# zhenxuan00/graphical-gan

Hardware: AMD Instinct MI355X
Metric: images/sec (G+D+GP step) cifar10 32x32 bs=64 (higher is better)
Workload: dtype f32; 1 GPU; gan_inference_cifar10.py MODE=wali-gp BATCH_SIZE=64 (per GPU) 32x32x3, CRITIC_ITERS=5; parallelism=dp1, global_batch=64, hip_graph=True, minibatch_feed=device-resident ring, read in place; one graph per iteration, finite_costs=True

## Files before the change

graphical_gan_amd/_lib.py:

```python
import ctypes as C
import os

_HERE = os.path.dirname(os.path.abspath(__file__))
LIB_PATH = os.path.join(_HERE, 'libggan.so')

ACT_NONE, ACT_LRELU, ACT_RELU, ACT_TANH, ACT_SIGMOID = 0, 1, 2, 3, 4
PACK_MAX = 64
HEAD_BCE_MAX_ROWS = 2048
BCE_HEADS = 2
PACK_ARRIVE_INTS = 33 * 1024
POSTERIOR_MAX_K = 8192
MODE_K = {'CONCRETE': 0, 'STRAIGHT_THROUGHT_CONCRETE': 1, 'STRAIGHT_THROUGHT': 2}
BCE_MAX = 16
TSNE_MAX_K = 128
TSNE_MAX_SPLITS = 64
ABI_VERSION = 800


class ConvGeom(C.Structure):
    _fields_ = [(n, C.c_int) for n in ('N', 'Ci', 'H', 'W', 'Co', 'Ho', 'Wo', 'k', 'stride', 'pad_t', 'pad_l',
                                       'plan_wgs', 'plan_wgs_filter', 'plan_flags')]


PLAN_PLAIN = 1
# ... 58 lines not shown
    'ggan_ssim_pairs_workspace': (_Z, [_I, _I, _I, _I]),
    'ggan_ssim_pairs': (_I, [_P, _P, _I, _I, _I, _I, _F, _F, _F, _F, _P, _P, _P, _Z, _P]),
    'ggan_noise_fill': (_I, [_P, _P, _P, _P, _P, _P, _I, _P, _P]),
    'ggan_gmm_latent_fwd': (_I, [_P, _P, _P, _P, _P, _I, _I, _I, _F, _F, _P]),
    'ggan_gmm_latent_bwd': (_I, [_P, _P, _P, _P, _P, _P, _P, _I, _I, _I, _F, _P]),
    'ggan_gmm_latent_st_fwd': (_I, [_P, _P, _P, _P, _P, _P, _I, _I, _I, _F, _F, _I, _P]),
    'ggan_gmm_latent_st_bwd': (_I, [_P, _P, _P, _P, _P, _P, _P, _I, _I, _I, _F, _I, _P]),
    'ggan_gmm_posterior_assign': (_I, [_P, _P, _F, _I, _I, _I, _I, _P, _P, _P, _P]),
    'ggan_cluster_accuracy': (_I, [_P, _P, _P, _I, _I, _P, _P]),
    'ggan_video_sheet_u8': (_I, [_P, _P, _P, _P, _I, _I, _I, _I, _I, _I, _I, _I, _I, _F, _F, _F, _P]),
    'ggan_tsne_sqnorms': (_I, [_P, _I, _I, _P, _P]),
    'ggan_tsne_neighbours': (_I, [_P, _P, _I, _I, _I, _I, _I, _P, _P, _P, _P, _Z, _P]),
    'ggan_tsne_affinities': (_I, [_P, _I, _I, _F, _I, _F, _P, _P, _P]),
    'ggan_tsne_symmetrise': (_I, [_P, _P, _I, _I, _P, _P, _P, _P, _P]),
    'ggan_tsne_gradient': (_I, [_P, _P, _P, _P, _I, _I, _P, _P, _P, _P, _P, _P]),
    'ggan_tsne_kl': (_I, [_P, _P, _P, _P, _I, _I, _P, _P, _P, _P, _P]),
    'ggan_tsne_iterate': (_I, [_P, _P, _P, _P, _P, _P, _P, _I, _I, _P, _P, _I, _I, _I, _F, _F, _F, _F, _F, _P]),
    'ggan_gemm_split': (_I, [_I, _I, _I, _I, _I, _P, _P, _I, _P, _P, _P, _P, _I, _P, _I, _F, _P, _Z, _P]),
    'ggan_gemm_colsum': (_I, [_I, _I, _I, _I, _P, _P, _P, _P, _P, _Z, _P]),
    'ggan_dyn_scan_fwd': (_I, [_I, _I, _I, _I, _I, _P, _P, _P, _P, _P, _P, _P, _P, _P, _P, _F, _P, _P, _P, _P]),
    'ggan_dyn_scan_bwd': (_I, [_I, _I, _I, _I, _I, _P, _P, _P, _P, _P, _P, _P, _P, _P, _F, _P, _P, _P, _P, _P, _P, _P]),
    'ggan_critic_head_fwd': (_I, [_I, _I, _I, _I, _P, _P, _P, _P, _P, _P, _F, _P, _P, _P, _Z, _P]),
    'ggan_critic_head_bwd': (_I, [_I, _I, _I, _I, _P, _P, _P, _P, _P, _P, _F, _P, _P, _P, _P, _P, _P, _P, _P, _Z, _P]),
    'ggan_critic_head_fwd_bce': (_I, [_I, _I, _I, _I, _P, _P, _P, _P, _P, _P, _F, _P, _P, _I, _I, _P, _P, _P, _P, _P, _P, _Z, _P]),
    'ggan_critic_head_bwd_tail': (_I, [_I, _I, _I, _I, _P, _P, _P, _P, _P, _F, _P, _P, _P, _P, _P, _P, _P, _P, _P, _I, _I, _P, _P, _P, _P, _P, _P, _Z, _P]),
    'ggan_linear_bwd_data_act': (_I, [_I, _I, _I, _P, _P, _I, _F, _P, _P, _P, _Z, _P]),
    'ggan_linear_bwd_weight_act': (_I, [_I, _I, _I, _P, _P, _P, _I, _F, _P, _P, _P, _Z, _P]),
    'ggan_colsum': (_I, [_P, _P, _I, _I, _P]),
    'ggan_reparam_fwd': (_I, [_P, _P, _P, _P, _P, _Z, _P]),
    'ggan_reparam_bwd': (_I, [_P, _P, _P, _P, _P, _P, _Z, _P]),
    'ggan_agg_div_fwd': (_I, [_I, _P, _P, _P, _P, _P, _I, _I, _I, _I, _P, _P, _P, _P, _P, _P]),
    'ggan_agg_div_bwd': (_I, [_I, _P, _P, _P, _P, _I, _I, _I, _I, _P, _P, _P, _P, _P, _P, _P, _P, _P]),
    'ggan_colsum_tall': (_I, [_P, _P, _I, _I, _P, _Z, _P]),
    'ggan_chansum': (_I, [_P, _P, _I, _I, _I, _P, _Z, _P]),
    'ggan_bn_fwd_train': (_I, [_P, _P, _P, _P, _P, _P, _I, _I, _I, _F, _I, _F, _P]),
    'ggan_bn_bwd': (_I, [_P, _P, _P, _P, _P, _P, _P, _P, _I, _I, _I, _P]),
    'ggan_bn_bwd_act': (_I, [_P, _P, _P, _I, _F, _P, _P, _P, _P, _P, _P, _P, _I, _I, _I, _P]),
    'ggan_bn_bwd_bwd': (_I, [_P, _P, _P, _I, _F, _P, _P, _P, _P, _P, _P, _P, _I, _I, _I, _P]),
    'ggan_bn_split_fwd_train': (_I, [_P, _P, _P, _P, _P, _P, _I, _I, _I, _I, _F, _I, _F, _P, _Z, _P]),
    'ggan_bn_split_bwd_act': (_I, [_P, _P, _I, _F, _P, _P, _P, _P, _P, _P, _P, _P, _I, _I, _I, _I, _I, _P, _Z, _P]),
    'ggan_bn_sync_stats': (_I, [_P, _P, _I, _I, _I, _P]),
    'ggan_bn_sync_apply': (_I, [_P, _P, _I, _P, _P, _P, _P, _P, _I, _I, _I, _F, _I, _F, _P]),
    'ggan_bn_sync_bwd_stats': (_I, [_P, _P, _P, _I, _F, _P, _P, _P, _I, _I, _I, _P]),
    'ggan_bn_sync_bwd_apply': (_I, [_P, _P, _P, _I, _F, _P, _P, _P, _P, _I, _I, _P, _P, _P, _I, _I, _I, _P]),
    'ggan_act_fwd': (_I, [_P, _P, _Z, _I, _F, _P]),
    'ggan_act_bwd': (_I, [_P, _P, _P, _Z, _I, _F, _P]),
    'ggan_act_bwd_chansum': (_I, [_P, _P, _P, _P, _I, C.POINTER(_I), _I, _I, _I, _I, _F, _P]),
    'ggan_bias_add': (_I, [_P, _P, _P, _I, _I, _I, _P]),
    'ggan_cast_scale_i32': (_I, [_P, _P, _P, _Z, _F, _F, _P]),
    'ggan_cast_scale_ring_i32': (_I, [_P, _I, _P, _P, _I, _P, _P, _Z, _F, _F, _P]),
    'ggan_axpby': (_I, [_P, _P, _P, _Z, _F, _F, _F, _P]),
    'ggan_mix_mean': (_I, [_P, _P, _P, _P, _I, _I, _I, _P]),
    'ggan_row_lerp': (_I, [_P, _P, _P, _P, _I, _I, _P]),
    'ggan_bce_logits_fwd': (_I, [_P, _F, _F, _P, _I, _I, _P]),
    'ggan_bce_logits_bwd': (_I, [_P, _F, _F, _P, _P, _I, _P]),
    'ggan_bce_logits_multi_fwd': (_I, [C.POINTER(_P), C.POINTER(_F), C.POINTER(_F), C.POINTER(_I), _I, _P, _P]),
    'ggan_bce_logits_multi_bwd': (_I, [C.POINTER(_P), C.POINTER(_F), C.POINTER(_F), C.POINTER(_I), _I, _P, C.POINTER(_P), _P]),
    'ggan_bce_logits_multi_fwd_grad': (_I, [C.POINTER(_P), C.POINTER(_F), C.POINTER(_F), C.POINTER(_I), _I, _P, C.POINTER(_P), _P]),
    'ggan_bce_head_bwd': (_I, [C.POINTER(_P), C.POINTER(_F), C.POINTER(_F), C.POINTER(_I), _I, _P, C.POINTER(_P), _I, _I, _P, _P, _F, _P, _P,
                          _P, _P]),
    'ggan_bce_heads_bwd': (_I, [C.POINTER(_P), C.POINTER(_F), C.POINTER(_F), C.POINTER(_I), _I, _P, C.POINTER(_P), _I, C.POINTER(_I),
                           C.POINTER(_I), C.POINTER(_I), C.POINTER(_P), C.POINTER(_P), C.POINTER(_F), C.POINTER(_P), C.POINTER(_P),
                           C.POINTER(_P), _P]),
    'ggan_mean_fwd': (_I, [_P, _F, _P, _I, _I, _P]),
    'ggan_mean_bwd': (_I, [_P, _F, _P, _I, _P]),
    'ggan_mean_multi_fwd_grad': (_I, [C.POINTER(_P), C.POINTER(_F), C.POINTER(_I), _I, _P, C.POINTER(_P), _P]),
    'ggan_dist_fwd': (_I, [_P, _P, _P, _Z, _I, _F, _I, _P]),
    'ggan_dist_bwd': (_I, [_P, _P, _P, _P, _P, _Z, _I, _F, _P]),
    'ggan_gp_penalty_fwd': (_I, [_P, _P, _P, _I, _I, _F, _P]),
    'ggan_gp_penalty_bwd': (_I, [_P, _P, _P, _P, _I, _I, _F, _P]),
    'ggan_gp_penalty_fwd_grad': (_I, [_P, _P, _P, _P, _P, _I, _I, _F, _P]),
    'ggan_adam_step': (_I, [_P, _P, _P, _P, _Z, _P, _F, _F, _F, _F, _F, _P]),
    'ggan_adam_advance': (_I, [_P, _P]),
    'ggan_rmsprop_step': (_I, [_P, _P, _P, _Z, _F, _F, _F, _F, _F, _F, _P]),
    'ggan_adam_step_counted': (_I, [_P, _P, _P, _P, _Z, _P, _F, _F, _F, _F, _F, _P]),
    'ggan_ema_step': (_I, [_P, _P, _Z, _P, _F, _P]),
    'ggan_swap': (_I, [_P, _P, _Z, _P]),
    'ggan_pack': (_I, [C.POINTER(_P), C.POINTER(_Z), C.POINTER(_Z), _I, _P, _P]),
    'ggan_pack_parts': (_I, [C.POINTER(_P), C.POINTER(_Z), C.POINTER(_Z), C.POINTER(_I), C.POINTER(_Z), _I, _P, _P, _P]),
    'ggan_pack_parts2': (_I, [C.POINTER(_P), C.POINTER(_Z), C.POINTER(_Z), C.POINTER(_I), C.POINTER(_Z), C.POINTER(_P), C.POINTER(_I),
                              C.POINTER(_Z), _I, _P, _P, _P]),
    'ggan_pack_adam': (_I, [C.POINTER(_P), C.POINTER(_Z), C.POINTER(_Z), C.POINTER(_I), C.POINTER(_Z), C.POINTER(_P), C.POINTER(_I),
                            C.POINTER(_Z), _I, _P, _P, _P, _P, _P, _P, _F, _F, _F, _F, _F, _P]),
    'ggan_prof_enable': (_I, [_I]),
    'ggan_prof_reset': (_I, []),
    'ggan_prof_report': (_I, [C.POINTER(ProfRec), _I]),
}

_lib = None


def load():
    global _lib
    if _lib is not None:
        return _lib
    if not os.path.exists(LIB_PATH):
        raise GganError('libggan.so not found at %s -- run `python -c "import __graft_entry__ as g; g.build()"` '
                        '(there is no CPU fallback)' % LIB_PATH)
    lib = C.CDLL(LIB_PATH)
    for name, (res, args) in SIGNATURES.items():
        try:
            fn = getattr(lib, name)
        except AttributeError:
            raise GganError('libggan.so does not export %s' % name)
        fn.restype = res
        fn.argtypes = args
# ... 24 lines not shown
```

graphical_gan_amd/build.py:

```python
import hashlib
import os
import subprocess
import sys

HERE = os.path.dirname(os.path.abspath(__file__))
CSRC = os.path.join(HERE, 'csrc')
LIB = os.path.join(HERE, 'libggan.so')
STAMP = os.path.join(HERE, '.libggan.stamp')
SOURCES = ['runtime.hip', 'pointwise.hip', 'bn.hip', 'linear_bn.hip', 'gemm.hip', 'conv_naive.hip', 'conv_corr.hip', 'conv_dg16.hip', 'conv_wgrad.hip', 'conv_wgrad_split.hip', 'conv_thin.hip', 'conv_api.hip', 'conv3d.hip', 'dynscan.hip', 'video_sheet.hip', 'tsne.hip', 'mmd_sets.hip', 'knn_sets.hip', 'knn_lists.hip', 'parzen_sets.hip', 'ssim_pairs.hip']
FLAGS = ['--offload-arch=gfx950', '-O3', '-std=c++17', '-fPIC', '-ffp-contract=on', '-Wall', '-Wno-unused-function']
EXTRA_FLAGS = {'conv_wgrad_split.hip': ['-mllvm', '-amdgpu-mfma-vgpr-form']}
if os.environ.get('GGAN_BUILD_DIAG'):
    FLAGS.append('-DGGAN_DIAG')


def _digest():
    h = hashlib.sha256()
    for root in (CSRC, os.path.join(HERE, '..', 'include')):
        for fn in sorted(os.listdir(root)):
            with open(os.path.join(root, fn), 'rb') as f:
                h.update(fn.encode())
                h.update(f.read())
    h.update(' '.join(FLAGS).encode())
    h.update(repr(sorted(EXTRA_FLAGS.items())).encode())
    return h.hexdigest()


def build_id():
    h = hashlib.sha256()
    try:
        with open(os.path.join(HERE, 'site_plans.json'), 'rb') as f:
            h.update(f.read())
    except OSError:
        pass
    return _digest()[:16] + '/' + h.hexdigest()[:8]


def build(force=False, verbose=False):
    import fcntl
    with open(os.path.join(HERE, '.libggan.lock'), 'w') as lock:
        fcntl.flock(lock, fcntl.LOCK_EX)
        try:
            return _build_locked(force, verbose)
        finally:
            fcntl.flock(lock, fcntl.LOCK_UN)


def _build_locked(force, verbose):
    dig = _digest()
    if not force and os.path.exists(LIB) and os.path.exists(STAMP) and open(STAMP).read().strip() == dig:
        return LIB
    hipcc = os.environ.get('HIPCC', '/opt/rocm/bin/hipcc')
    objs = []
    procs = []
    for src in SOURCES:
        obj = os.path.join(HERE, 'build', src.replace('.hip', '.o'))
        os.makedirs(os.path.dirname(obj), exist_ok=True)
        cmd = [hipcc] + FLAGS + EXTRA_FLAGS.get(src, []) + ['-c', os.path.join(CSRC, src), '-o', obj]
        if verbose:
            print(' '.join(cmd))
        procs.append((src, subprocess.Popen(cmd, stdout=subprocess.PIPE, stderr=subprocess.STDOUT)))
        objs.append(obj)
# ... 22 lines not shown
```

graphical_gan_amd/functional/__init__.py:

```python

from ._core import (
    C, os, weakref, torch, Function, once_differentiable, _lib, ACT_NONE, ACT_LRELU, ACT_RELU, ACT_TANH, ACT_SIGMOID, ConvGeom,
    check, _WS, _WS_BYTES, _L, _p, _stream, _dev, _c, _DEFER, _DATA_ONLY, _is_param, data_grad_only,
    _skip_undefined, defer_wgrad_reduce, _wgrad_parts, _STREAMS, shared_stream, workspace, _PLAN, _PLAIN, _SERIAL_BWD, target_workgroups,
    launch_hint, serial_backward, _remembers_plan, force_plain,
    same_geometry, conv_geom, _geom, _SITE, site_scope, site_plan, RowSlot, _new_out, _adjacent, HEAD_LOGITS, _PENDING_COSTS, _tail_value, settle_cost,
    pending_costs, drop_pending_costs, UNIT_SEEDS, unit_seed, is_unit_seed, LATE_EXT, _LATE_TERMS, mark_ready, wait_ready, add_late_terms,
    drop_late_terms)
from .pointwise import ActFwd, ActBwd, leaky_relu, relu, tanh, sigmoid
from .conv import (
    DEBUG_POISON_CHECK, PendingCast, ConvFwd, _fused_conv_backward, ConvDgrad, ConvDgradMasked, ConvWgrad, ChanSum, TALL_ROWS,
    ColSum)
from .linear import (
    Gemm, _fused_linear_backward, Gemm2, _CONSTS, cached_const, Gemm2Dgrad, _HEAD_HINT, head_bce_hint, CriticHead, DynScan,
    gemm_colsum_, linear)
from .norm import BatchNormTrain, BatchNormGroupedTrain, BatchNormBwd, LinearBatchNormRows, _all_gather_rows, SyncBatchNormTrain
from .rows import (
    JoinRows, Fanout, fanout, SplitRows, CastScaleI32, Axpby, MixMean, GmmLatent, GmmLatentST, MixRbfMmd2, MixRbfMmd2Unbiased, mix_rbf_sums, mmd2_from_sums, MMD_FUSED_MAX_ROWS, knn_radii, ball_counts, prdc, PRDC_MAX_K, knn_lists, knn_vote, knn_accuracy, KNN_MAX_K, KNN_MAX_CLASSES, parzen_lse, parzen_ll, PARZEN_MAX_SIGMAS, ssim_pairs, psnr_from_mse, Reparam, AGG_KL, AGG_IKL, AGG_JSD,
    AggDiv, RowLerp, gmm_posterior_assign_, cluster_accuracy_, sheet_grid, video_sheet_u8)
from .conv3d import _dims3, Im2Col3d, Col2Im3d, _conv3d_patch, _igemm_ok, Conv3dImplicit, conv3d
from .losses import BceSum, Distance, MeanSum, GradPenalty
from .optim_ops import ema_step_, swap_
from .optim_ops import adam_step_, rmsprop_step_, NOISE_NORMAL, NOISE_UNIFORM, NOISE_ONEHOT, noise_state, noise_fill_, pack_
from .tsne import (
    tsne, tsne_splits, tsne_neighbours, tsne_affinities, tsne_symmetrise, tsne_gradient, tsne_kl, tsne_step, tsne_affinity_graph)
```

graphical_gan_amd/functional/linear.py:

```python
import ctypes as C
import os
import threading as _threading
import torch
import weakref
from .. import _lib
from torch.autograd import Function
from torch.autograd.function import once_differentiable
from .._lib import ACT_NONE, check
from ._core import (
    _L, _p, _stream, _c, _DATA_ONLY, _is_param, _skip_undefined, workspace, _new_out, HEAD_LOGITS, _PENDING_COSTS,
    _tail_value)
from .pointwise import ActBwd
from .conv import TALL_ROWS, ColSum


@_skip_undefined
class Gemm(Function):

    @staticmethod
    def forward(ctx, a, b, bias, ta, tb, act, alpha, slot=None):
        a, b = _c(a), _c(b)
        M, K = (a.shape[1], a.shape[0]) if ta else (a.shape[0], a.shape[1])
        K2, N = (b.shape[1], b.shape[0]) if tb else (b.shape[0], b.shape[1])
        assert K == K2, (a.shape, b.shape, ta, tb)
# ... 123 lines not shown

_CONSTS = {}


def cached_const(value, shape, device):
    device = torch.device(device)
    key = (float(value), tuple(shape), device.type, device.index)
    t = _CONSTS.get(key)
    if t is None:
        t = _CONSTS[key] = torch.full(tuple(shape), float(value), dtype=torch.float32, device=device)
    return t


class Gemm2Dgrad(Function):

    @staticmethod
    def forward(ctx, g, w, K1):
        g, w = _c(g), _c(w)
        M, N = g.shape
        K = w.shape[0]
        da1 = torch.empty((M, K1), dtype=torch.float32, device=g.device)
        da2 = torch.empty((M, K - K1), dtype=torch.float32, device=g.device)
        ws = workspace(g.device)
        check(_L().ggan_gemm_split(0, 1, M, K, N, _p(g), _p(None), 0, _p(w), _p(None), _p(da1), _p(da2), K1, _p(None), ACT_NONE, 0.0,
                                   _p(ws), ws.numel(), _stream()), 'ggan_gemm_split')
        ctx.K1 = K1
        ctx.w_param = _is_param(w)
        ctx.set_materialize_grads(False)
        ctx.save_for_backward(g, w)
        return da1, da2

    @staticmethod
    def backward(ctx, h1, h2):
        if h1 is None and h2 is None:
            return None, None, None
        g, w = ctx.saved_tensors
        K1 = ctx.K1
        M, N = g.shape
        K = w.shape[0]
        h1 = _c(h1) if h1 is not None else cached_const(0.0, (M, K1), g.device)
        h2 = _c(h2) if h2 is not None else cached_const(0.0, (M, K - K1), g.device)
        dg = dw = None
        if ctx.needs_input_grad[0]:
            dg = Gemm2.apply(h1, h2, w, None, ACT_NONE, 0.0)
        if ctx.needs_input_grad[1] and not (_DATA_ONLY[0] and ctx.w_param):
            if torch.is_grad_enabled():
                dw = Gemm.apply(torch.cat([h1, h2], 1), g, None, True, False, ACT_NONE, 0.0)
            else:
                dw = torch.empty((K, N), dtype=torch.float32, device=g.device)
                ws = workspace(g.device)
                check(_L().ggan_gemm_split(1, 0, K, N, M, _p(h1), _p(h2), K1, _p(g), _p(None), _p(dw), _p(None), 0, _p(None), ACT_NONE,
                                           0.0, _p(ws), ws.numel(), _stream()), 'ggan_gemm_split')
        return dg, dw, None


_HEAD_HINT = _threading.local()


class head_bce_hint(object):

    def __init__(self, terms, kind='bce'):
        self.terms = (kind, tuple((int(n), float(z), float(w)) for n, z, w in terms)) if terms else None

    def __enter__(self):
        self.prev = getattr(_HEAD_HINT, 'terms', None)
        _HEAD_HINT.terms = self.terms
        return self

    def __exit__(self, *exc):
        _HEAD_HINT.terms = self.prev
        return False


@_skip_undefined
class CriticHead(Function):

    @staticmethod
    def forward(ctx, a1, a2, w, b, w_out, b_out, alpha):
        a1, w, b, w_out, b_out = _c(a1), _c(w), _c(b), _c(w_out), _c(b_out)
        a2 = _c(a2) if a2 is not None else None
        M, K1 = a1.shape
        K2 = a2.shape[1] if a2 is not None else 0
        H = w.shape[1]
        assert w.shape[0] == K1 + K2 and w_out.numel() == H and b.numel() == H, (a1.shape, w.shape, w_out.shape)
        h = torch.empty((M, H), dtype=torch.float32, device=a1.device)
        logits = torch.empty((M,), dtype=torch.float32, device=a1.device)
        ws = workspace(a1.device)
        registers = M <= _lib.HEAD_BCE_MAX_ROWS and any(ctx.needs_input_grad) and not os.environ.get('GGAN_NO_HEAD_BCE')
        hint = getattr(_HEAD_HINT, 'terms', None)
        hinted = None
        hkind, hterms = hint if hint is not None else (None, ())
        if (registers and hint is not None and 1 <= len(hterms) <= 3 and sum(n for n, _, _ in hterms) == M and H <= 2048
                and not os.environ.get('GGAN_NO_HEAD_HINT')):
            g = torch.empty((M,), dtype=torch.float32, device=a1.device)
            gh = torch.empty((M, H), dtype=torch.float32, device=a1.device)
            nt = len(hterms)
            tabs = ((C.c_int * nt)(*[n for n, _, _ in hterms]), (C.c_float * nt)(*[z for _, z, _ in hterms]),
                    (C.c_float * nt)(*[wt for _, _, wt in hterms]))
            check(_L().ggan_critic_head_fwd_bce(M, K1, K2, H, _p(a1), _p(a2), _p(w), _p(b), _p(w_out), _p(b_out), float(alpha), _p(h),
                                                _p(logits), 1 if hkind == 'mean' else 0, nt, tabs[0], tabs[1], tabs[2], _p(g), _p(gh), _p(ws),
                                                ws.numel(), _stream()), 'ggan_critic_head_fwd_bce')
            hinted = dict(kind=hkind, terms=hterms, g=g, gh=gh)
        else:
            check(_L().ggan_critic_head_fwd(M, K1, K2, H, _p(a1), _p(a2), _p(w), _p(b), _p(w_out), _p(b_out), float(alpha), _p(h),
                                            _p(logits), _p(ws), ws.numel(), _stream()), 'ggan_critic_head_fwd')
        ctx.alpha, ctx.has_a2 = float(alpha), a2 is not None
# ... 123 lines not shown
```

graphical_gan_amd/models.py:

```python
import contextlib
import os
import weakref

import numpy as np
import torch

from . import functional as F
from . import tflib as lib
from .tflib.ops.act import LRELU, RELU, TANH, SIGMOID

NETS_TARGET_WGS = 128
GP_TARGET_WGS = 128


class Config(object):
    def __init__(self, dataset='cifar10', batch_size=64, n_coms=0, mode=None, dim=None, dim_latent=128, bn=None,
                 temp=0.1, fuse=True, lr=None, batch_critic=True, mode_k='CONCRETE'):
        self.dataset, self.B, self.K, self.dim_latent, self.temp, self.fuse = dataset, batch_size, n_coms, dim_latent, temp, fuse
        assert mode_k in ('CONCRETE', 'STRAIGHT_THROUGHT_CONCRETE', 'STRAIGHT_THROUGHT'), mode_k
        self.mode_k = mode_k
        if dataset == 'cifar10':
            self.C, self.S, self.dim, self.nl, self.bn, self.out_act = 3, 32, 64, 3, True, 'tanh'
        elif dataset == 'svhn':
            self.C, self.S, self.dim, self.nl, self.bn, self.out_act = 3, 32, 64, 3, False, 'tanh'
# ... 158 lines not shown
            out = self._bn('Generator.BN1', [0], out, RELU)
        else:
            out = self._lin('Generator.Input', c.dim_latent, c.flat, noise, RELU)
        slot = out_slot
        out = out.reshape(-1, c.top, 4, 4)
        names = ['2', '3', '4', '5'] if c.nl == 4 else ['2', '3', '5']
        ch = c.top
        for i, nm in enumerate(names):
            last = i == len(names) - 1
            cout = c.C if last else ch // 2
            final_act = TANH if c.out_act == 'tanh' else SIGMOID
            if last:
                if c.fuse:
                    out = lib.ops.deconv2d.Deconv2D('Generator.' + nm, ch, cout, 5, out, activation=final_act, out=slot)
                else:
                    out = F.ActFwd.apply(lib.ops.deconv2d.Deconv2D('Generator.' + nm, ch, cout, 5, out), final_act, 0.0)
            elif c.bn:
                out = lib.ops.deconv2d.Deconv2D('Generator.' + nm, ch, cout, 5, out)
                out = self._bn('Generator.BN' + nm, [0, 2, 3], out, RELU)
            elif c.fuse:
                out = lib.ops.deconv2d.Deconv2D('Generator.' + nm, ch, cout, 5, out, activation=RELU)
            else:
                out = F.relu(lib.ops.deconv2d.Deconv2D('Generator.' + nm, ch, cout, 5, out))
            if c.dataset == 'mnist' and nm == '2':
                out = out[:, :, :7, :7].contiguous()
            ch = cout
        return out.reshape(-1, c.output_dim)

    def Extractor(self, inputs, out_slot=None, eps=None, after_first=None):
        c = self.cfg
        out = inputs.reshape(-1, c.C, c.S, c.S)
        ch = c.C
        for i in range(c.nl):
            cout = c.dim * 2 ** i
            name = 'Extractor.%d' % (i + 1)
            if c.bn and i > 0:
                out = lib.ops.conv2d.Conv2D(name, ch, cout, 5, out, stride=2)
                out = self._bn('Extractor.BN%d' % (i + 1), [0, 2, 3], out, LRELU)
            else:
                out = self._conv(name, ch, cout, out, LRELU)
            if i == 0 and after_first is not None:
                after_first()
            ch = cout
        out = out.reshape(-1, c.flat)
        if eps is not None:
            log_std = lib.ops.linear.Linear('Extractor.Std', c.flat, c.dim_latent, out)
            mean = lib.ops.linear.Linear('Extractor.Output', c.flat, c.dim_latent, out)
            z, std = F.Reparam.apply(mean, log_std, eps)
            return z, mean, std
        return lib.ops.linear.Linear('Extractor.Output', c.flat, c.dim_latent, out, out=out_slot)

    def Discriminator(self, x, z, grad_rows=None, twice=False, before_z=None, z_out=None):
        c = self.cfg
        out = x.reshape(-1, c.C, c.S, c.S)
        ch = c.C
        for i in range(c.nl):
            cout = c.dim * 2 ** i
            name = 'Discriminator.%d' % (i + 1)
            if c.critic_deep and c.bn and i > 0:
                out = lib.ops.conv2d.Conv2D(name, ch, cout, 5, out, stride=2, grad_rows=grad_rows)
                out = self._bn('Discriminator.BN%d' % (i + 1), [0, 2, 3], out, LRELU)
            else:
                out = self._conv(name, ch, cout, out, LRELU, grad_rows)
            ch = cout
        out = out.reshape(-1, c.flat)
        self._critic_features = weakref.ref(out)
        if before_z is not None:
            before_z()
        if z_out is None:
            z_out = self._lin('Discriminator.z1', c.dim_latent, 512, z, LRELU)
        if c.critic_deep:
            z_out = self._lin('Discriminator.2', 512, 512, z_out, LRELU)
            out = self._lin('Discriminator.zx1', c.flat + 512, 512, (out, z_out), LRELU)
            if c.fuse:
                return lib.ops.linear.LinearLReLULinear('Discriminator.zx2', 512, 512, 'Discriminator.Output', out, differentiable=twice)
            out = self._lin('Discriminator.zx2', 512, 512, out, LRELU)
            return lib.ops.linear.Linear('Discriminator.Output', 512, 1, out).reshape(-1)
        if c.fuse:
            return lib.ops.linear.LinearLReLULinear('Discriminator.zx1', c.flat + 512, 512, 'Discriminator.Output', (out, z_out),
                                                    differentiable=twice)
        out = self._lin('Discriminator.zx1', c.flat + 512, 512, (out, z_out), LRELU)
        out = lib.ops.linear.Linear('Discriminator.Output', 512, 1, out)
        return out.reshape(-1)

    def LatentDiscriminator(self, z, noise):
        c = self.cfg
        out = F.Axpby.apply(z, noise[0], 1.0, 0.3, 0.0)
        for i, (nm, nin, nout) in enumerate([('Input', c.dim_latent, 1024), ('2', 1024, 512), ('3', 512, 256), ('4', 256, 256)]):
            if c.bn:
                out = lib.ops.linear.Linear('Discriminator.' + nm, nin, nout, out)
                out = self._bn('Discriminator.BN%d' % (i + 1), [0], out, LRELU)
            else:
                out = self._lin('Discriminator.' + nm, nin, nout, out, LRELU)
            if i < 3:
                out = F.Axpby.apply(out, noise[i + 1], 1.0, 0.5, 0.0)
        return lib.ops.linear.Linear('Discriminator.Output', 256, 1, out).reshape(-1)

    def _forward_latent(self, feed, which, out):
        c = self.cfg
        real_x, q_z, p_z = out['real_x'], out['q_z'], out['p_z']
        J = lib.objs.gan_inference
        J.ONLY[0] = which
        noise = lambda tag: [feed['dn_%s%d' % (tag, i)] for i in range(4)]
        det = (lambda t: t.detach()) if which == 'disc' else (lambda t: t)
        with (lib.frozen('Discriminator') if which == 'gen' else lib.frozen()):
            d_real = self.LatentDiscriminator(p_z, noise('r'))
            d_fake = self.LatentDiscriminator(det(q_z), noise('f'))
            gp = None
            if c.mode == 'vegan-wgan-gp' and which != 'gen':
                z_hat = F.RowLerp.apply(p_z, det(q_z), feed['alpha'])
                if not z_hat.requires_grad:
                    z_hat.requires_grad_(True)
                d_hat = self.LatentDiscriminator(z_hat, noise('h'))
                with F.data_grad_only():
                    (g,) = torch.autograd.grad(d_hat, [z_hat], grad_outputs=F.cached_const(1.0, d_hat.shape, d_hat.device), create_graph=True)
                gp = F.GradPenalty.apply(g, 10.0)
        rec = 1. * lib.utils.distance.distance(real_x, self.Generator(q_z), 'l2') if which != 'disc' else None
        gen_params, disc_params = self._var_lists()
        if c.mode == 'vegan':
            res = J.vegan(d_fake, d_real, rec, gen_params, disc_params, c.lamb, lr=c.lr, beta1=c.beta1)
        else:
            res = J.vegan_wgan_gp(d_fake, d_real, rec, gp, gen_params, disc_params, c.lamb, lr=c.lr, beta1=c.beta1)
        J.ONLY[0] = None
        out.update(disc_fake=d_fake, disc_real=d_real, rec_penalty=rec, gradient_penalty=gp, gen_cost=res[0], disc_cost=res[1],
                   gen_train_op=res[2], disc_train_op=res[3])
        return out

    def HyperDiscriminator(self, z, k):
        c = self.cfg
        out = self._lin('Discriminator.HyperInput', c.dim_latent + c.K, 512, (z, k), LRELU)
        out = self._lin('Discriminator.Hyper2', 512, 512, out, LRELU)
        if c.fuse:
            return lib.ops.linear.LinearLReLULinear('Discriminator.Hyper3', 512, 512, 'Discriminator.HyperOutput', out)
        out = self._lin('Discriminator.Hyper3', 512, 512, out, LRELU)
        out = lib.ops.linear.Linear('Discriminator.HyperOutput', 512, 1, out)
        return out.reshape(-1)
# ... 189 lines not shown
                fl, rl = (1.0, 0.0) if which == 'gen' else (0.0, 1.0)
                hint = [(c.B, fl, 1.0), (c.B, rl, 1.0)]
            elif c.mode == 'local_ep' and c.K:
                fl, rl = (1.0, 0.0) if which == 'gen' else (0.0, 1.0)
                hint = [(c.B, fl, 0.5), (c.B, rl, 0.5)]
            elif c.mode == 'wali-gp' and not c.K:
                sg = -1.0 if which == 'gen' else 1.0
                hint, hkind = [(c.B, 0.0, sg), (c.B, 0.0, -sg)], 'mean'
        with (lib.frozen('Discriminator') if which == 'gen' else lib.frozen()), F.head_bce_hint(hint, hkind):
            d_fake, d_real = self._critic(batched, real_x, q_z, p_z, fake_x, onehot if c.K else None, q_k if c.K else None,
                                          detach=which == 'disc')
        if gp_early is not None and not late_gp:
            torch.cuda.current_stream(real_x.device).wait_stream(self._gp_stream)
        gen_params, disc_params = self._var_lists()
        rec_penalty = None
        if which != 'disc' and c.mode in ('alice', 'alice-z', 'alice-x', 'local_epce'):
            D = lib.utils.distance.distance
            if c.mode != 'alice-x':
                rec_penalty = 1. * D(real_x, self.Generator(q_z), 'l2')
            if c.mode in ('alice', 'alice-x'):
                rz = 1. * D(p_z, self.Extractor(fake_x), 'l2')
                rec_penalty = rz if rec_penalty is None else rec_penalty + rz
            out['rec_penalty'] = rec_penalty
        if c.mode == 'local_epce':
            res = J.local_epce(d_fake, d_real, rec_penalty, gen_params, disc_params, lr=c.lr, beta1=c.beta1)
        elif c.mode.startswith('alice'):
            res = J.alice(d_fake, d_real, rec_penalty, gen_params, disc_params, lr=c.lr, beta1=c.beta1)
        elif c.K:
            res = J.local_ep(d_fake, d_real, gen_params, disc_params, lr=c.lr, beta1=c.beta1)
        elif c.mode == 'wali':
            r = J.wali(d_fake, d_real, gen_params, disc_params)
            res = (r[0], r[1], r[3], r[4])
        elif c.mode == 'wali-gp':
            if which == 'gen':
                gp = None
            else:
                gp = gp_early if gp_early is not None else self._penalty(J, batched, real_x, fake_x, q_z, p_z, feed)
            F.LATE_EXT[0] = late_gp and gp is gp_early and gp is not None
            try:
                res = J.wali_gp(d_fake, d_real, gp, gen_params, disc_params)
            finally:
                F.LATE_EXT[0] = False
            out['gradient_penalty'] = gp
        else:
            res = J.ali(d_fake, d_real, gen_params, disc_params, lr=c.lr, beta1=c.beta1)
        J.ONLY[0] = None
        out.update(disc_fake=d_fake, disc_real=d_real, gen_cost=res[0], disc_cost=res[1],
                   gen_train_op=res[2], disc_train_op=res[3])
        return out

    def _penalty(self, J, batched, real_x, fake_x, q_z, p_z, feed):
        with (lib.second_leaf() if batched else lib.frozen()):
            return J.gradient_penalty(lambda xx, zz: self.Discriminator(xx, zz, twice=True), real_x, fake_x.detach() if batched else fake_x,
                                      q_z.detach() if batched else q_z, p_z.detach() if batched else p_z, feed['alpha'])

    def _critic(self, batched, real_x, q_z, p_z, fake_x, onehot, q_k, detach=True):
        c = self.cfg
        if not batched:
            if c.K:
                return ([self.HyperDiscriminator(p_z, onehot), self.Discriminator(fake_x, p_z)],
                        [self.HyperDiscriminator(q_z, q_k), self.Discriminator(real_x, q_z)])
            return self.Discriminator(fake_x, p_z), self.Discriminator(real_x, q_z)
        if detach:
            fake_x, p_z, q_z = fake_x.detach(), p_z.detach(), q_z.detach()
            q_k = q_k.detach() if c.K else None
        B = fake_x.shape[0]
        assert detach or not real_x.requires_grad, 'batched critic with grad_rows: real_x must not require a gradient'
        self.join_side(x_only=True)
        x_cat, z_cat = F.JoinRows.apply(fake_x, real_x), F.JoinRows.apply(p_z, q_z)
        z_cat, z_cat_h = F.fanout(z_cat, 2) if (c.K and c.fuse) else (z_cat, z_cat)
        z_out = None
        pj = self._pending_join
        gp_on_side = self._gp_stream is not None and self.cfg.mode == 'wali-gp' and detach and self.fork_now
        if pj is not None and not gp_on_side:
            with torch.cuda.stream(self._side):
                self._side.wait_event(self._noise_event)
                z_out = self._lin('Discriminator.z1', c.dim_latent, 512, z_cat, LRELU)
                ev = torch.cuda.Event()
                ev.record(self._side)
                pj[2] = ev
        fork_h = bool(c.K) and self.fork_nets and self.fork_now and x_cat.is_cuda
        if fork_h:
            cur = torch.cuda.current_stream(x_cat.device)
            if pj is None:
                self.join_side()
                self._side.wait_stream(cur)
            ev_z = torch.cuda.Event()
            with torch.cuda.stream(self._side):
                if z_out is None:
                    z_out = self._lin('Discriminator.z1', c.dim_latent, 512, z_cat, LRELU)
                    ev_z.record(self._side)
                else:
                    ev_z = None
                h = self.HyperDiscriminator(z_cat_h, F.JoinRows.apply(onehot, q_k))
            before = (lambda: cur.wait_event(ev_z)) if ev_z is not None else self.join_side
            d = self.Discriminator(x_cat, z_cat, grad_rows=None if detach else B, before_z=before, z_out=z_out)
        else:
            d = self.Discriminator(x_cat, z_cat, grad_rows=None if detach else B, before_z=self.join_side, z_out=z_out)
        if fork_h:
            cur.wait_stream(self._side)
        elif c.K:
            h = self.HyperDiscriminator(z_cat_h, F.JoinRows.apply(onehot, q_k))
        if c.K:
            (hf, hr), (df, dr) = F.SplitRows.apply(h, B), F.SplitRows.apply(d, B)
            return [hf, df], [hr, dr]
        return F.SplitRows.apply(d, B)
```

graphical_gan_amd/tflib/objs/gan_inference.py:

```python
import numpy as np

from ... import functional as F
from ...optim import TrainOp, get_optimizer


ONLY = [None]
_val = F.settle_cost


def _bce_costs(fakes, reals, ratios):
    logits, gl, dl, w = [], [], [], []
    for f, r, ratio in zip(fakes, reals, ratios):
        logits += [f, r]
        gl += [1.0, 0.0]
        dl += [0.0, 1.0]
        w += [float(ratio), float(ratio)]
    gen_cost = F.BceSum.apply(tuple(gl), tuple(w), *logits) if ONLY[0] != 'disc' else None
    disc_cost = F.BceSum.apply(tuple(dl), tuple(w), *logits) if ONLY[0] != 'gen' else None
    return gen_cost, disc_cost


def ali(disc_fake, disc_real, gen_params, disc_params, lr=2e-4, beta1=0.5, beta2=0.999, s_f=None):
    gen_cost, disc_cost = _bce_costs([disc_fake], [disc_real], [1.0])
    if s_f is not None and gen_cost is not None:
# ... 70 lines not shown
    gen_opt = get_optimizer('gen', gen_params, lr=lr, beta1=beta1, beta2=0.999)
    disc_opt = get_optimizer('disc', disc_params, lr=lr, beta1=beta1, beta2=0.999)
    return gen_cost, disc_cost, TrainOp(gen_opt, gen_cost), TrainOp(disc_opt, disc_cost)


def local_ep_dynamic(disc_fake_zz, disc_real_zz, disc_fake_xz, disc_real_xz, gen_params, disc_params, lr=2e-4, beta1=0.5, beta2=.999,
                     rec_penalty=None):
    n = len(disc_fake_zz)
    assert n == len(disc_real_zz)
    w = 1.0 / (n + 1) if n > 0 else 1.0
    gen_cost, disc_cost = _bce_costs(list(disc_fake_zz) + [disc_fake_xz], list(disc_real_zz) + [disc_real_xz], [w] * n + [1.0])
    gen_cost = _plus(gen_cost, rec_penalty)
    gen_opt = get_optimizer('gen', gen_params, lr=lr, beta1=beta1, beta2=beta2)
    disc_opt = get_optimizer('disc', disc_params, lr=lr, beta1=beta1, beta2=beta2)
    return gen_cost, disc_cost, TrainOp(gen_opt, gen_cost), TrainOp(disc_opt, disc_cost)


def weighted_local_epce(disc_fake_list, disc_real_list, ratio_list, gen_params, disc_params, lr=2e-4, beta1=0.5,
                        rec_penalty=None):
    ratio_list = np.asarray(ratio_list)
    assert len(disc_fake_list) == ratio_list.shape[0]
    gen_cost, disc_cost = _bce_costs(disc_fake_list, disc_real_list, list(ratio_list))
    gen_debug_list, disc_debug_list = [], []
    if rec_penalty is not None and gen_cost is not None:
        gen_cost = _val(gen_cost) + rec_penalty
    gen_opt = get_optimizer('gen', gen_params, lr=lr, beta1=beta1, beta2=0.999)
    disc_opt = get_optimizer('disc', disc_params, lr=lr, beta1=beta1, beta2=0.999)
    return (gen_cost, disc_cost, gen_debug_list, disc_debug_list,
            TrainOp(gen_opt, gen_cost), TrainOp(disc_opt, disc_cost))


def wali(disc_fake, disc_real, gen_params, disc_params, lr=5e-5):
    gen_cost = F.MeanSum.apply((-1.0, -1.0), disc_fake, disc_real) if ONLY[0] != 'disc' else None
    disc_cost = F.MeanSum.apply((1.0, -1.0), disc_fake, disc_real) if ONLY[0] != 'gen' else None
    gen_opt = get_optimizer('gen', gen_params, kind='rmsprop', lr=lr)
    disc_opt = get_optimizer('disc', disc_params, kind='rmsprop', lr=lr, clip=(-.01, .01))
    noop = lambda: None
    return gen_cost, disc_cost, noop, TrainOp(gen_opt, gen_cost), TrainOp(disc_opt, disc_cost), [noop]


def wali_gp(disc_fake, disc_real, gradient_penalty, gen_params, disc_params, lr=1e-4):
    gen_cost = F.MeanSum.apply((-1.0, 1.0), disc_fake, disc_real) if ONLY[0] != 'disc' else None
    disc_cost = None
    if ONLY[0] != 'gen':
        if gradient_penalty is not None:
            disc_cost = F.MeanSum.apply((1.0, -1.0, 1.0), disc_fake, disc_real, gradient_penalty)
        else:
            disc_cost = F.MeanSum.apply((1.0, -1.0), disc_fake, disc_real)
    gen_opt = get_optimizer('gen', gen_params, lr=lr, beta1=0.5, beta2=0.9)
    disc_opt = get_optimizer('disc', disc_params, lr=lr, beta1=0.5, beta2=0.9)
    return gen_cost, disc_cost, TrainOp(gen_opt, gen_cost), TrainOp(disc_opt, disc_cost)


def gradient_penalty(critic, real_x, fake_x, q_z, p_z, alpha, lam=10.):
    import torch
    x_hat = F.RowLerp.apply(real_x, fake_x, alpha)
    z_hat = F.RowLerp.apply(q_z, p_z, alpha)
    if not x_hat.requires_grad:
        x_hat.requires_grad_(True)
    d_hat = critic(x_hat, z_hat)
    ones = F.cached_const(1.0, d_hat.shape, d_hat.device)
    with F.data_grad_only():
        (g,) = torch.autograd.grad(d_hat, [x_hat], grad_outputs=ones, create_graph=True)
    return F.GradPenalty.apply(g.reshape(g.shape[0], -1), float(lam))
```

include/ggan.h:

```cpp
#ifndef GGAN_H
#define GGAN_H
#include <stddef.h>
#include <stdint.h>

#ifdef __cplusplus
extern "C" {
#endif

typedef void* ggan_stream_t;
#define GGAN_WS_RESERVED 16384

enum { GGAN_ACT_NONE = 0, GGAN_ACT_LRELU = 1, GGAN_ACT_RELU = 2, GGAN_ACT_TANH = 3, GGAN_ACT_SIGMOID = 4 };

#define GGAN_ABI_VERSION 800
int ggan_version(void);
const char* ggan_last_error(void);
typedef struct {
    int N, Ci, H, W;
    int Co, Ho, Wo;
    int k, stride, pad_t, pad_l;
    int plan_wgs, plan_wgs_filter, plan_flags;
} ggan_conv_geom;
#define GGAN_PLAN_PLAIN 1

// ... 200 lines not shown
int ggan_agg_div_fwd(int kind, const float* mu, const float* sd, const float* k_onehot, const float* eps_q, const float* z_p, int nx, int nz,
                     int d, int n_coms, float* out, float* Z, float* A, float* Bv, float* T, ggan_stream_t stream);
int ggan_agg_div_bwd(int kind, const float* mu, const float* sd, const float* k_onehot, const float* eps_q, int nx, int nz, int d, int n_coms,
                     const float* Z, const float* A, const float* Bv, const float* gout, float* W, float* GZ, float* gmu, float* gsd,
                     ggan_stream_t stream);

#define GGAN_NOISE_MAX 16
int ggan_noise_fill(float* const* dsts, const size_t* sizes, const int* kinds, const float* a, const float* b, const int* widths,
                    int count, uint64_t* state, ggan_stream_t stream);
int ggan_gmm_latent_fwd(const float* z, const float* mu, const float* gumbel_u, float* logits, float* k, int B, int K, int D,
                        float log_pi, float temp, ggan_stream_t stream);
int ggan_gmm_latent_bwd(const float* z, const float* mu, const float* k, const float* g_logits, const float* g_k, float* dz,
                        float* dmu, int B, int K, int D, float temp, ggan_stream_t stream);
enum { GGAN_MODE_K_CONCRETE = 0, GGAN_MODE_K_STC = 1, GGAN_MODE_K_ST = 2 };
int ggan_gmm_latent_st_fwd(const float* z, const float* mu, const float* gumbel_u, float* logits, float* k, float* soft, int B, int K,
                           int D, float log_pi, float temp, int mode, ggan_stream_t stream);
int ggan_gmm_latent_st_bwd(const float* z, const float* mu, const float* soft, const float* g_logits, const float* g_k, float* dz,
                           float* dmu, int B, int K, int D, float temp, int mode, ggan_stream_t stream);
#define GGAN_POSTERIOR_MAX_K 8192
int ggan_gmm_posterior_assign(const float* z, const float* mu, float log_pi, int B, int K, int D, int row0, float* probs,
                              int32_t* assign, uint64_t* colbest, ggan_stream_t stream);
int ggan_cluster_accuracy(const int32_t* assign, const int32_t* labels, const uint64_t* colbest, int N, int K, int32_t* correct,
                          ggan_stream_t stream);
int ggan_video_sheet_u8(const float* gen, const float* data, uint8_t* sheet, uint8_t* gif, int n, int rows, int LEN, int C, int H, int W,
                        int nh, int nw, int interleave, float a, float b, float d, ggan_stream_t stream);

#define GGAN_TSNE_MAX_K 128
#define GGAN_TSNE_MAX_SPLITS 64
int ggan_tsne_sqnorms(const float* x, int N, int D, float* norms, ggan_stream_t stream);
int ggan_tsne_neighbours(const float* x, const float* norms, int N, int D, int row0, int rows, int K, float* dots, int32_t* idx, float* dist,
                         void* ws, size_t ws_bytes, ggan_stream_t stream);
int ggan_tsne_affinities(const float* dist, int N, int K, float perplexity, int steps, float tol, float* p_cond, float* beta,
                         ggan_stream_t stream);
int ggan_tsne_symmetrise(const int32_t* idx, const float* p_cond, int N, int K, int* ptr, int32_t* col, float* val, int* scratch,
                         ggan_stream_t stream);
int ggan_tsne_gradient(const int* ptr, const int32_t* col, const float* val, const float* y, int N, int splits, float* part, float* zblk,
                       float* attr, float* rep, float* z, ggan_stream_t stream);
int ggan_tsne_kl(const int* ptr, const int32_t* col, const float* val, const float* y, int N, int splits, float* part, float* zblk,
                 float* klrow, float* kl, ggan_stream_t stream);
int ggan_tsne_iterate(const int* ptr, const int32_t* col, const float* val, float* ya, float* yb, float* vel, float* gains, int N, int splits,
                      float* part, float* zblk, int it0, int it1, int exploration_iters, float early_exaggeration, float momentum0,
                      float momentum1, float learning_rate, float min_gain, ggan_stream_t stream);

int ggan_dist_fwd(const float* x, const float* y, float* out, size_t n, int p, float weight, int accumulate,
                  ggan_stream_t stream);
int ggan_dist_bwd(const float* x, const float* y, const float* gout, float* gx, float* gy, size_t n, int p,
                  float weight, ggan_stream_t stream);
int ggan_gp_penalty_fwd(const float* g, float* slopes, float* pen, int B, int D, float lam,
                        ggan_stream_t stream);
int ggan_gp_penalty_bwd(const float* g, const float* slopes, const float* gpen, float* gg, int B, int D,
                        float lam, ggan_stream_t stream);
int ggan_gp_penalty_fwd_grad(const float* g, float* slopes, float* pen, float* gg_unit, int32_t* arrive, int B, int D, float lam,
                             ggan_stream_t stream);

int ggan_adam_step(float* theta, const float* g, float* m, float* v, size_t n, const int32_t* step,
                   float lr, float beta1, float beta2, float eps, float grad_scale, ggan_stream_t stream);
int ggan_adam_advance(int32_t* step, ggan_stream_t stream);

int ggan_rmsprop_step(float* theta, const float* g, float* ms, size_t n, float lr, float decay, float eps,
                      float grad_scale, float clip_lo, float clip_hi, ggan_stream_t stream);
int ggan_adam_step_counted(float* theta, const float* g, float* m, float* v, size_t n, const int32_t* step, float lr,
                           float beta1, float beta2, float eps, float grad_scale, ggan_stream_t stream);
int ggan_ema_step(float* shadow, const float* theta, size_t n, const int32_t* step, float decay, ggan_stream_t stream);
int ggan_swap(float* a, float* b, size_t n, ggan_stream_t stream);
#define GGAN_PACK_MAX 64
int ggan_pack(const float* const* srcs, const size_t* sizes, const size_t* offsets, int count,
              float* flat, ggan_stream_t stream);
int ggan_pack_parts(const float* const* srcs, const size_t* sizes, const size_t* offsets, const int* parts,
                    const size_t* strides, int count, float* flat, int32_t* bump, ggan_stream_t stream);
int ggan_pack_parts2(const float* const* srcs, const size_t* sizes, const size_t* offsets, const int* parts, const size_t* strides,
                     const float* const* srcs2, const int* parts2, const size_t* strides2, int count, float* flat, int32_t* bump,
                     ggan_stream_t stream);
#define GGAN_PACK_ARRIVE_STRIDE 1024
#define GGAN_PACK_ARRIVE_INTS (33 * GGAN_PACK_ARRIVE_STRIDE)
int ggan_pack_adam(const float* const* srcs, const size_t* sizes, const size_t* offsets, const int* parts, const size_t* strides,
                   const float* const* srcs2 , const int* parts2, const size_t* strides2, int count, float* flat,
                   float* theta, float* m, float* v, int32_t* step, int32_t* arrive, float lr, float beta1, float beta2, float eps,
                   float grad_scale, ggan_stream_t stream);

typedef struct { char name[48]; double total_ms; long launches; double flops; double bytes; long grid; } ggan_prof_rec;
int ggan_prof_enable(int on);
int ggan_prof_reset(void);
int ggan_prof_report(ggan_prof_rec* out, int cap);

#ifdef __cplusplus
}
#endif
#endif
```

Before: 17230 images/sec.

## Compute gradient-penalty head input gradient analytically with a fused seed kernel

Adds a custom HeadInputGrad function that computes the critic head's forward activation and its input gradient directly: a GEMM, then an elementwise seed kernel (w_out times the LReLU derivative), then a transposed GEMM. The gradient penalty uses it instead of running the full critic head and differentiating it through autograd. This removes the head's output layer and the autograd double-backward graph for the penalty, and the second-order backward through the head is written by hand. The hand-written backward is complex and a wrong term would go unnoticed. The path can be disabled with an environment variable.

```diff
diff --git a/graphical_gan_amd/_lib.py b/graphical_gan_amd/_lib.py
--- a/graphical_gan_amd/_lib.py
+++ b/graphical_gan_amd/_lib.py
@@ -134,6 +134,7 @@
     'ggan_axpby': (_I, [_P, _P, _P, _Z, _F, _F, _F, _P]),
     'ggan_mix_mean': (_I, [_P, _P, _P, _P, _I, _I, _I, _P]),
     'ggan_row_lerp': (_I, [_P, _P, _P, _P, _I, _I, _P]),
+    'ggan_head_seed_fwd': (_I, [_I, _I, _P, _P, _P, _F, _P, _P]),
     'ggan_bce_logits_fwd': (_I, [_P, _F, _F, _P, _I, _I, _P]),
     'ggan_bce_logits_bwd': (_I, [_P, _F, _F, _P, _P, _I, _P]),
     'ggan_bce_logits_multi_fwd': (_I, [C.POINTER(_P), C.POINTER(_F), C.POINTER(_F), C.POINTER(_I), _I, _P, _P]),
diff --git a/graphical_gan_amd/build.py b/graphical_gan_amd/build.py
--- a/graphical_gan_amd/build.py
+++ b/graphical_gan_amd/build.py
@@ -7,7 +7,7 @@
 CSRC = os.path.join(HERE, 'csrc')
 LIB = os.path.join(HERE, 'libggan.so')
 STAMP = os.path.join(HERE, '.libggan.stamp')
-SOURCES = ['runtime.hip', 'pointwise.hip', 'bn.hip', 'linear_bn.hip', 'gemm.hip', 'conv_naive.hip', 'conv_corr.hip', 'conv_dg16.hip', 'conv_wgrad.hip', 'conv_wgrad_split.hip', 'conv_thin.hip', 'conv_api.hip', 'conv3d.hip', 'dynscan.hip', 'video_sheet.hip', 'tsne.hip', 'mmd_sets.hip', 'knn_sets.hip', 'knn_lists.hip', 'parzen_sets.hip', 'ssim_pairs.hip']
+SOURCES = ['runtime.hip', 'pointwise.hip', 'penalty_tail.hip', 'bn.hip', 'linear_bn.hip', 'gemm.hip', 'conv_naive.hip', 'conv_corr.hip', 'conv_dg16.hip', 'conv_wgrad.hip', 'conv_wgrad_split.hip', 'conv_thin.hip', 'conv_api.hip', 'conv3d.hip', 'dynscan.hip', 'video_sheet.hip', 'tsne.hip', 'mmd_sets.hip', 'knn_sets.hip', 'knn_lists.hip', 'parzen_sets.hip', 'ssim_pairs.hip']
 FLAGS = ['--offload-arch=gfx950', '-O3', '-std=c++17', '-fPIC', '-ffp-contract=on', '-Wall', '-Wno-unused-function']
 EXTRA_FLAGS = {'conv_wgrad_split.hip': ['-mllvm', '-amdgpu-mfma-vgpr-form']}
 if os.environ.get('GGAN_BUILD_DIAG'):
diff --git a/graphical_gan_amd/csrc/penalty_tail.hip b/graphical_gan_amd/csrc/penalty_tail.hip
--- /dev/null
+++ b/graphical_gan_amd/csrc/penalty_tail.hip
@@ -0,0 +1,60 @@
+#include "common.h"
+using namespace ggan;
+
+namespace {
+
+__device__ __forceinline__ float seed1(float s, float w, float r, float alpha) {
+    const float g = s * w + 0.f;
+    return act_grad(g, r, GGAN_ACT_LRELU, alpha);
+}
+
+__global__ void head_seed_fwd4_k(const float* __restrict__ u, const float* __restrict__ h, const float* __restrict__ w_out,
+                                 float* __restrict__ gpre, unsigned total4, unsigned H4, float alpha) {
+    const unsigned stride = gridDim.x * blockDim.x;
+    const float4* h4 = reinterpret_cast<const float4*>(h);
+    const float4* w4 = reinterpret_cast<const float4*>(w_out);
+    float4* o4 = reinterpret_cast<float4*>(gpre);
+    for (unsigned i = blockIdx.x * blockDim.x + threadIdx.x; i < total4; i += stride) {
+        const unsigned n = i / H4, j4 = i - n * H4;
+        const float s = u ? u[n] : 1.f;
+        const float4 w = w4[j4], r = h4[i];
+        float4 o;
+        o.x = seed1(s, w.x, r.x, alpha); o.y = seed1(s, w.y, r.y, alpha);
+        o.z = seed1(s, w.z, r.z, alpha); o.w = seed1(s, w.w, r.w, alpha);
+        o4[i] = o;
+    }
+}
+
+__global__ void head_seed_fwd1_k(const float* __restrict__ u, const float* __restrict__ h, const float* __restrict__ w_out,
+                                 float* __restrict__ gpre, unsigned total, unsigned H, float alpha) {
+    const unsigned stride = gridDim.x * blockDim.x;
+    for (unsigned i = blockIdx.x * blockDim.x + threadIdx.x; i < total; i += stride) {
+        const unsigned n = i / H, j = i - n * H;
+        gpre[i] = seed1(u ? u[n] : 1.f, w_out[j], h[i], alpha);
+    }
+}
+
+inline bool aligned16(const void* p) { return ((uintptr_t)p & 15) == 0; }
+
+}
+
+extern "C" {
+
+int ggan_head_seed_fwd(int M, int H, const float* u, const float* h, const float* w_out, float alpha, float* gpre, ggan_stream_t stream) {
+    GGAN_CHECK_ARG(h && w_out && gpre, "null pointer");
+    GGAN_CHECK_ARG(M >= 1 && H >= 1 && (double)M * H < 2147483648.0, "bad shape");
+    const unsigned total = (unsigned)M * (unsigned)H;
+    if ((H & 3) == 0 && aligned16(h) && aligned16(w_out) && aligned16(gpre)) {
+        const unsigned total4 = total / 4;
+        const int grid = (int)((total4 + 255) / 256 < 2048 ? (total4 + 255) / 256 : 2048);
+        GGAN_LAUNCH("head_seed_fwd", 1.0 * total, 8.0 * total, head_seed_fwd4_k, dim3(grid), dim3(256), 0, (hipStream_t)stream, u, h, w_out, gpre,
+                    total4, (unsigned)(H / 4), alpha);
+        return 0;
+    }
+    const int grid = (int)((total + 255) / 256 < 2048 ? (total + 255) / 256 : 2048);
+    GGAN_LAUNCH("head_seed_fwd", 1.0 * total, 8.0 * total, head_seed_fwd1_k, dim3(grid), dim3(256), 0, (hipStream_t)stream, u, h, w_out, gpre, total,
+                (unsigned)H, alpha);
+    return 0;
+}
+
+}
diff --git a/graphical_gan_amd/functional/__init__.py b/graphical_gan_amd/functional/__init__.py
--- a/graphical_gan_amd/functional/__init__.py
+++ b/graphical_gan_amd/functional/__init__.py
@@ -12,7 +12,7 @@
     DEBUG_POISON_CHECK, PendingCast, ConvFwd, _fused_conv_backward, ConvDgrad, ConvDgradMasked, ConvWgrad, ChanSum, TALL_ROWS,
     ColSum)
 from .linear import (
-    Gemm, _fused_linear_backward, Gemm2, _CONSTS, cached_const, Gemm2Dgrad, _HEAD_HINT, head_bce_hint, CriticHead, DynScan,
+    Gemm, _fused_linear_backward, Gemm2, _CONSTS, cached_const, Gemm2Dgrad, HeadInputGrad, _HEAD_HINT, head_bce_hint, CriticHead, DynScan,
     gemm_colsum_, linear)
 from .norm import BatchNormTrain, BatchNormGroupedTrain, BatchNormBwd, LinearBatchNormRows, _all_gather_rows, SyncBatchNormTrain
 from .rows import (
diff --git a/graphical_gan_amd/functional/linear.py b/graphical_gan_amd/functional/linear.py
--- a/graphical_gan_amd/functional/linear.py
+++ b/graphical_gan_amd/functional/linear.py
@@ -199,6 +199,58 @@
                 check(_L().ggan_gemm_split(1, 0, K, N, M, _p(h1), _p(h2), K1, _p(g), _p(None), _p(dw), _p(None), 0, _p(None), ACT_NONE,
                                            0.0, _p(ws), ws.numel(), _stream()), 'ggan_gemm_split')
         return dg, dw, None
+
+
+@_skip_undefined
+class HeadInputGrad(Function):
+
+    @staticmethod
+    def forward(ctx, a1, a2, w, b, w_out, alpha):
+        a1, a2, w, w_out = _c(a1), _c(a2), _c(w), _c(w_out)
+        M, K1, K2 = a1.shape[0], a1.shape[1], a2.shape[1]
+        K, H = w.shape
+        assert K == K1 + K2 and a2.shape[0] == M and w_out.numel() == H, (a1.shape, a2.shape, w.shape, w_out.shape)
+        dev = a1.device
+        new = lambda *shape: torch.empty(shape, dtype=torch.float32, device=dev)
+        L, ws = _L(), workspace(dev)
+        h, gpre, d_a1, d_a2 = new(M, H), new(M, H), new(M, K1), new(M, K2)
+        check(L.ggan_gemm_split(0, 0, M, H, K, _p(a1), _p(a2), K1, _p(w), _p(_c(b)) if b is not None else _p(None), _p(h), _p(None), 0,
+                                _p(None), _lib.ACT_LRELU, float(alpha), _p(ws), ws.numel(), _stream()), 'ggan_gemm_split')
+        check(L.ggan_head_seed_fwd(M, H, _p(None), _p(h), _p(w_out), float(alpha), _p(gpre), _stream()), 'ggan_head_seed_fwd')
+        check(L.ggan_gemm_split(0, 1, M, K, H, _p(gpre), _p(None), 0, _p(w), _p(None), _p(d_a1), _p(d_a2), K1, _p(None), ACT_NONE, 0.0,
+                                _p(ws), ws.numel(), _stream()), 'ggan_gemm_split')
+        ctx.alpha, ctx.K1 = float(alpha), K1
+        ctx.w_param, ctx.wout_param = _is_param(w), _is_param(w_out)
+        ctx.save_for_backward(h, gpre, w, w_out)
+        return d_a1
+
+    @staticmethod
+    @once_differentiable
+    def backward(ctx, hh1):
+        h, gpre, w, w_out = ctx.saved_tensors
+        hh1 = _c(hh1)
+        M, H = h.shape
+        K, K1 = w.shape[0], ctx.K1
+        dev = h.device
+        zero = cached_const(0.0, (M, K - K1), dev)
+        L, ws = _L(), workspace(dev)
+        d_w = d_wout = None
+        if ctx.needs_input_grad[4] and not (_DATA_ONLY[0] and ctx.wout_param):
+            t = torch.empty((M, H), dtype=torch.float32, device=dev)
+            check(L.ggan_gemm_split(0, 0, M, H, K, _p(hh1), _p(zero), K1, _p(w), _p(None), _p(t), _p(None), 0, _p(None), ACT_NONE, 0.0,
+                                    _p(ws), ws.numel(), _stream()), 'ggan_gemm_split')
+        if ctx.needs_input_grad[2] and not (_DATA_ONLY[0] and ctx.w_param):
+            d_w = torch.empty((K, H), dtype=torch.float32, device=dev)
+            check(L.ggan_gemm_split(1, 0, K, H, M, _p(hh1), _p(zero), K1, _p(gpre), _p(None), _p(d_w), _p(None), 0, _p(None), ACT_NONE, 0.0,
+                                    _p(ws), ws.numel(), _stream()), 'ggan_gemm_split')
+        if ctx.needs_input_grad[4] and not (_DATA_ONLY[0] and ctx.wout_param):
+            mt = torch.empty_like(t)
+            check(L.ggan_act_bwd(_p(t), _p(h), _p(mt), t.numel(), _lib.ACT_LRELU, ctx.alpha, _stream()), 'ggan_act_bwd')
+            d_wout = torch.empty((H, 1), dtype=torch.float32, device=dev)
+            check(L.ggan_gemm(1, 0, H, 1, M, _p(mt), _p(cached_const(1.0, (M, 1), dev)), _p(None), _p(d_wout), ACT_NONE, 0.0, _p(ws),
+                              ws.numel(), _stream()), 'ggan_gemm')
+            d_wout = d_wout.view(w_out.shape)
+        return None, None, d_w, None, d_wout, None
 
 
 _HEAD_HINT = _threading.local()
diff --git a/graphical_gan_amd/models.py b/graphical_gan_amd/models.py
--- a/graphical_gan_amd/models.py
+++ b/graphical_gan_amd/models.py
@@ -234,6 +234,34 @@
 
     def Discriminator(self, x, z, grad_rows=None, twice=False, before_z=None, z_out=None):
         c = self.cfg
+        out, z_out = self._critic_stack(x, z, grad_rows, before_z, z_out)
+        if c.critic_deep:
+            z_out = self._lin('Discriminator.2', 512, 512, z_out, LRELU)
+            out = self._lin('Discriminator.zx1', c.flat + 512, 512, (out, z_out), LRELU)
+            if c.fuse:
+                return lib.ops.linear.LinearLReLULinear('Discriminator.zx2', 512, 512, 'Discriminator.Output', out, differentiable=twice)
+            out = self._lin('Discriminator.zx2', 512, 512, out, LRELU)
+            return lib.ops.linear.Linear('Discriminator.Output', 512, 1, out).reshape(-1)
+        if c.fuse:
+            return lib.ops.linear.LinearLReLULinear('Discriminator.zx1', c.flat + 512, 512, 'Discriminator.Output', (out, z_out),
+                                                    differentiable=twice)
+        out = self._lin('Discriminator.zx1', c.flat + 512, 512, (out, z_out), LRELU)
+        out = lib.ops.linear.Linear('Discriminator.Output', 512, 1, out)
+        return out.reshape(-1)
+
+    def penalty_seed_ok(self):
+        c = self.cfg
+        return c.fuse and not c.critic_deep and c.flat % 64 == 0 and not os.environ.get('GGAN_NO_PENALTY_SEED')
+
+    def DiscriminatorInputGrad(self, x, z):
+        c = self.cfg
+        a1, z_out = self._critic_stack(x, z)
+        w, b = lib.ops.linear.linear_params('Discriminator.zx1', c.flat + 512, 512)
+        w_out, _ = lib.ops.linear.linear_params('Discriminator.Output', 512, 1)
+        return a1, F.HeadInputGrad.apply(a1, z_out, w, b, w_out, 0.2)
+
+    def _critic_stack(self, x, z, grad_rows=None, before_z=None, z_out=None):
+        c = self.cfg
         out = x.reshape(-1, c.C, c.S, c.S)
         ch = c.C
         for i in range(c.nl):
@@ -251,19 +279,7 @@
             before_z()
         if z_out is None:
             z_out = self._lin('Discriminator.z1', c.dim_latent, 512, z, LRELU)
-        if c.critic_deep:
-            z_out = self._lin('Discriminator.2', 512, 512, z_out, LRELU)
-            out = self._lin('Discriminator.zx1', c.flat + 512, 512, (out, z_out), LRELU)
-            if c.fuse:
-                return lib.ops.linear.LinearLReLULinear('Discriminator.zx2', 512, 512, 'Discriminator.Output', out, differentiable=twice)
-            out = self._lin('Discriminator.zx2', 512, 512, out, LRELU)
-            return lib.ops.linear.Linear('Discriminator.Output', 512, 1, out).reshape(-1)
-        if c.fuse:
-            return lib.ops.linear.LinearLReLULinear('Discriminator.zx1', c.flat + 512, 512, 'Discriminator.Output', (out, z_out),
-                                                    differentiable=twice)
-        out = self._lin('Discriminator.zx1', c.flat + 512, 512, (out, z_out), LRELU)
-        out = lib.ops.linear.Linear('Discriminator.Output', 512, 1, out)
-        return out.reshape(-1)
+        return out, z_out
 
     def LatentDiscriminator(self, z, noise):
         c = self.cfg
@@ -559,7 +575,8 @@
     def _penalty(self, J, batched, real_x, fake_x, q_z, p_z, feed):
         with (lib.second_leaf() if batched else lib.frozen()):
             return J.gradient_penalty(lambda xx, zz: self.Discriminator(xx, zz, twice=True), real_x, fake_x.detach() if batched else fake_x,
-                                      q_z.detach() if batched else q_z, p_z.detach() if batched else p_z, feed['alpha'])
+                                      q_z.detach() if batched else q_z, p_z.detach() if batched else p_z, feed['alpha'],
+                                      input_grad=self.DiscriminatorInputGrad if self.penalty_seed_ok() else None)
 
     def _critic(self, batched, real_x, q_z, p_z, fake_x, onehot, q_k, detach=True):
         c = self.cfg
diff --git a/graphical_gan_amd/tflib/objs/gan_inference.py b/graphical_gan_amd/tflib/objs/gan_inference.py
--- a/graphical_gan_amd/tflib/objs/gan_inference.py
+++ b/graphical_gan_amd/tflib/objs/gan_inference.py
@@ -146,12 +146,17 @@
     return gen_cost, disc_cost, TrainOp(gen_opt, gen_cost), TrainOp(disc_opt, disc_cost)
 
 
-def gradient_penalty(critic, real_x, fake_x, q_z, p_z, alpha, lam=10.):
+def gradient_penalty(critic, real_x, fake_x, q_z, p_z, alpha, lam=10., input_grad=None):
     import torch
     x_hat = F.RowLerp.apply(real_x, fake_x, alpha)
     z_hat = F.RowLerp.apply(q_z, p_z, alpha)
     if not x_hat.requires_grad:
         x_hat.requires_grad_(True)
+    if input_grad is not None:
+        a1, d_a1 = input_grad(x_hat, z_hat)
+        with F.data_grad_only():
+            (g,) = torch.autograd.grad(a1, [x_hat], grad_outputs=d_a1, create_graph=True)
+        return F.GradPenalty.apply(g.reshape(g.shape[0], -1), float(lam))
     d_hat = critic(x_hat, z_hat)
     ones = F.cached_const(1.0, d_hat.shape, d_hat.device)
     with F.data_grad_only():
diff --git a/include/ggan.h b/include/ggan.h
--- a/include/ggan.h
+++ b/include/ggan.h
@@ -276,6 +276,8 @@
                         float lam, ggan_stream_t stream);
 int ggan_gp_penalty_fwd_grad(const float* g, float* slopes, float* pen, float* gg_unit, int32_t* arrive, int B, int D, float lam,
                              ggan_stream_t stream);
+int ggan_head_seed_fwd(int M, int H, const float* u , const float* h, const float* w_out, float alpha, float* gpre,
+                       ggan_stream_t stream);
 
 int ggan_adam_step(float* theta, const float* g, float* m, float* v, size_t n, const int32_t* step,
                    float lr, float beta1, float beta2, float eps, float grad_scale, ggan_stream_t stream);
```

Measured after the change: 17450 images/sec (median of 6 runs). +1.3%, better.
